# dog-qiuqiu/Yolo-FastestV2

Hardware: AMD Instinct MI355X
Metric: images/sec at 352x352 bs=256 per GPU (forward+decode+NMS) (higher is better)
Workload: dtype f32 tensors; contractions fp16x3 (two-term fp16 split operands on v_mfma_f32_16x16x32_f16, fp32 accumulate); depthwise/BN/ReLU/decode/NMS fp32 VALU; 1 GPU

## Files before the change

yolo_fastestv2_amd/csrc/yfv2_stage2h.hip:

```cpp
#include "yfv2_internal.h"
#include <atomic>
#include <utility>

typedef _Float16 yfv2_h8 __attribute__((ext_vector_type(8)));
typedef _Float16 yfv2_h2 __attribute__((ext_vector_type(2)));

namespace {

__device__ __forceinline__ float row_shr1(float v) {
  return __builtin_bit_cast(float, __builtin_amdgcn_update_dpp(0, __builtin_bit_cast(int, v), 0x111, 0xf, 0xf, true));
}
__device__ __forceinline__ float row_shl1(float v) {
  return __builtin_bit_cast(float, __builtin_amdgcn_update_dpp(0, __builtin_bit_cast(int, v), 0x101, 0xf, 0xf, true));
}
template <int K>
__device__ __forceinline__ float quad_mul(float tap4, float v) {
  return __builtin_bit_cast(float, __builtin_amdgcn_update_dpp(0, __builtin_bit_cast(int, tap4), K * 0x55, 0xf, 0xf, false)) * v;
}
#define YFV2_QP(n) "quad_perm:[%" #n ",%" #n ",%" #n ",%" #n "] row_mask:0xf bank_mask:0xf\n\t"
template <int K3, int K4, int K5, int K6, int K7, int K8>
__device__ __forceinline__ void quad_fmac6(float& a0, float& a1, float& a2, float t3, float t4, float t5, float t6, float t7, float t8,
                                           float u, float w) {
  asm("s_nop 1\n\tv_fmac_f32_dpp %0, %3, %9 " YFV2_QP(11) "v_fmac_f32_dpp %1, %4, %9 " YFV2_QP(12) "v_fmac_f32_dpp %2, %5, %9 " YFV2_QP(13)
      "v_fmac_f32_dpp %0, %6, %10 " YFV2_QP(14) "v_fmac_f32_dpp %1, %7, %10 " YFV2_QP(15) "v_fmac_f32_dpp %2, %8, %10 " YFV2_QP(16)
      : "+v"(a0), "+v"(a1), "+v"(a2)
      : "v"(t3), "v"(t4), "v"(t5), "v"(t6), "v"(t7), "v"(t8), "v"(u), "v"(w), "n"(K3), "n"(K4), "n"(K5), "n"(K6), "n"(K7), "n"(K8));
}
template <int KA, int KB, int KC>
__device__ __forceinline__ void quad_fmac3(float& s, float& q, float ta, float tb, float tc, float v0, float v1) {
  asm("s_nop 1\n\tv_fmac_f32_dpp %0, %2, %5 " YFV2_QP(7) "v_fmac_f32_dpp %1, %3, %6 " YFV2_QP(8) "v_fmac_f32_dpp %0, %4, %6 " YFV2_QP(9)
      : "+v"(s), "+v"(q) : "v"(ta), "v"(tb), "v"(tc), "v"(v0), "v"(v1), "n"(KA), "n"(KB), "n"(KC));
}
template <int KA>
__device__ __forceinline__ void quad_fmac1(float& s, float ta, float v) {
  asm("s_nop 1\n\tv_fmac_f32_dpp %0, %1, %2 " YFV2_QP(3) : "+v"(s) : "v"(ta), "v"(v), "n"(KA));
}
#undef YFV2_QP
__device__ __forceinline__ void dpp_src_ready(float& v) { asm volatile("s_nop 1" : "+v"(v)); }

__device__ __forceinline__ void split2(f32x2 v, unsigned& h1, unsigned& h2) {
  const yfv2_h2 t1 = __builtin_convertvector(v, yfv2_h2);
  const f32x2 r = v - __builtin_convertvector(t1, f32x2);
  const yfv2_h2 t2 = __builtin_convertvector(r, yfv2_h2);
  h1 = __builtin_bit_cast(unsigned, t1);
  h2 = __builtin_bit_cast(unsigned, t2);
}
__device__ __forceinline__ void pw_h3(const yfv2_h8 (&w)[2][2], const f32x2 (&in)[4], const f32x4 (&init)[2], f32x4 (&acc)[2], Yfv2Watch& watch) {
  u32x4 b1, b2;
#pragma unroll
  for (int k = 0; k < 4; ++k) { unsigned h1, h2; split2(in[k], h1, h2); b1[k] = h1; b2[k] = h2; }
  const yfv2_h8 x1 = __builtin_bit_cast(yfv2_h8, b1), x2 = __builtin_bit_cast(yfv2_h8, b2);
#pragma unroll
  for (int t = 0; t < 2; ++t) acc[t] = __builtin_amdgcn_mfma_f32_16x16x32_f16(w[t][0], x2, init[t], 0, 0, 0);
#pragma unroll
  for (int t = 0; t < 2; ++t) acc[t] = __builtin_amdgcn_mfma_f32_16x16x32_f16(w[t][1], x1, acc[t], 0, 0, 0);
#pragma unroll
  for (int t = 0; t < 2; ++t) acc[t] = __builtin_amdgcn_mfma_f32_16x16x32_f16(w[t][0], x1, acc[t], 0, 0, 0);
  watch.see(acc[0][0]);
}

}

constexpr int S1H_W1 = 0, S1H_W2 = 1024, S1H_TAPS = 2048, S1H_CST = 3200, S1H_OFFS = 3272;

__global__ __launch_bounds__(64, 3) void s1h_kernel(S1PxArgs a) {
  const int H = a.H, W = a.W;
  const int nstrips = a.nstrips, nb = a.nb, R = a.R;
  const int wpi = nstrips * nb;
  const int nwg = gridDim.x;
  const int wid = (nwg & 7) ? (int)blockIdx.x : (int)(blockIdx.x & 7) * (nwg >> 3) + (int)(blockIdx.x >> 3);
  const int b = __builtin_amdgcn_readfirstlane(wid / wpi), wi = __builtin_amdgcn_readfirstlane(wid - b * wpi);
  const int strip = wi % nstrips, band = wi / nstrips;
  const int lane = threadIdx.x, l = lane & 15, g = lane >> 4;
  const int x = 14 * strip + l;
  const bool xok = x < W;
  const bool st_lane = xok && (l > 0 || strip == 0) && (l < 15 || strip == nstrips - 1);
  const int y0 = band * R, y1 = min(H, y0 + R);
  constexpr int OOB = (int)0x80000000;

  __amdgpu_buffer_rsrc_t rsrc = __builtin_amdgcn_make_buffer_rsrc((void*)(a.act + (size_t)b * a.img_stride), 0, a.num_records, 0x00020000);
  const float* img = a.img16;
  yfv2_h8 w1[2][2], w2[2][2];
  {
    const u32x4* q = reinterpret_cast<const u32x4*>(img);
#pragma unroll
    for (int t = 0; t < 2; ++t)
#pragma unroll
      for (int k = 0; k < 2; ++k) {
        w1[t][k] = __builtin_bit_cast(yfv2_h8, q[(S1H_W1 / 4) + (t * 2 + k) * 64 + lane]);
        w2[t][k] = __builtin_bit_cast(yfv2_h8, q[(S1H_W2 / 4) + (t * 2 + k) * 64 + lane]);
      }
  }
  Yfv2Watch watch;
  float tq[18];
#pragma unroll
  for (int q = 0; q < 18; ++q) tq[q] = img[S1H_TAPS + q * 64 + lane];
  const f32x4 sh1[2] = {*reinterpret_cast<const f32x4*>(img + S1H_CST + 4 * g), *reinterpret_cast<const f32x4*>(img + S1H_CST + 16 + 4 * g)};
  const f32x4 bi2[2] = {*reinterpret_cast<const f32x4*>(img + S1H_CST + 32 + 4 * g), *reinterpret_cast<const f32x4*>(img + S1H_CST + 48 + 4 * g)};
  const float unscale2 = img[S1H_CST + 64];
  int soff[4], doff[4];
  {
    const int* po = reinterpret_cast<const int*>(img + S1H_OFFS);
#pragma unroll
    for (int k = 0; k < 4; ++k) {
      const int so = po[k * 64 + lane], dd = po[(4 + k) * 64 + lane];
      soff[k] = (xok && so != OOB) ? so + x * 8 : OOB;
      doff[k] = (st_lane && dd != OOB) ? dd + x * 8 : OOB;
    }
  }
  const int rowb = W * 8;

  auto load_row = [&](int r, f32x2 (&v)[4]) {
    const bool rok = r >= 0 && r < H;
#pragma unroll
// ... 795 lines not shown
    }(std::make_integer_sequence<int, 12>{});
  };

  f32x4 X[6], Y[6];
  float cxe[12], cxo[12], cte[12], cto[12];
  {
    const int iy = 2 * y0 - 1;
    load_row(iy, X);
    load_row(iy + 1, Y);
    columns(X, (xok && iy >= 0) ? __builtin_inff() : 0.f, cxe, cxo, cte, cto);
    load_row(iy + 2, X);
  }
  const float limx = xok ? __builtin_inff() : 0.f;
  for (int j = 0; j < R; ++j) {
    const int oy = y0 + j;
    float Sm[12], Qm[12], Sp[12], Qp[12], xe[12], xo[12], te[12], to[12];
    {
      float tm[27], tp[27]; ld_taps(tm, tp);
      acc_row(std::integral_constant<int, 0>{}, tm, cte, cto, Sm, Qm);
      acc_row(std::integral_constant<int, 0>{}, tp, cxe, cxo, Sp, Qp);
    }
    columns(Y, limx, xe, xo, te, to);
    {
      float tm[27], tp[27]; ld_taps(tm, tp);
      acc_row(std::integral_constant<int, 1>{}, tm, te, to, Sm, Qm);
      acc_row(std::integral_constant<int, 1>{}, tp, xe, xo, Sp, Qp);
    }
    __builtin_amdgcn_sched_barrier(0);
    load_row(2 * oy + 2, Y);
    __builtin_amdgcn_sched_barrier(0);
    columns(X, limx, cxe, cxo, cte, cto);
    {
      float tm[27], tp[27]; ld_taps(tm, tp);
      acc_row(std::integral_constant<int, 2>{}, tm, cte, cto, Sm, Qm);
      acc_row(std::integral_constant<int, 2>{}, tp, cxe, cxo, Sp, Qp);
    }
    __builtin_amdgcn_sched_barrier(0);
    load_row(2 * oy + 3, X);
    __builtin_amdgcn_sched_barrier(0);
    f32x2 dm[6], dp[6];
#pragma unroll
    for (int c = 0; c < 12; ++c) {
      dpp_src_ready(Qm[c]); dpp_src_ready(Qp[c]);
      dm[c >> 1][c & 1] = Sm[c] + row_shr1(Qm[c]);
      dp[c >> 1][c & 1] = Sp[c] + row_shr1(Qp[c]);
    }
    f32x4 am[3], ap[3];
    { f32x4 bip[3]; ld_c3(48, bip); pw_h3_48(WP, lane, dp, bip, ap, watch); }
    { f32x4 bi2[3]; ld_c3(96, bi2); pw_h3_48(W2, lane, dm, bi2, am, watch); }
    if (st_lane && oy < y1) {
      float* o = outp + (size_t)oy * OW * 96;
#pragma unroll
      for (int t = 0; t < 3; ++t) {
        f32x4 vp, vm;
#pragma unroll
        for (int e = 0; e < 4; ++e) { vp[e] = __builtin_fmaxf(ap[t][e], 0.f) * unscale_p; vm[e] = __builtin_fmaxf(am[t][e], 0.f) * unscale_2; }
        *reinterpret_cast<f32x4*>(o + 16 * t) = vp;
        *reinterpret_cast<f32x4*>(o + 48 + 16 * t) = vm;
      }
    }
  }
  watch.report(a.nonfinite);
#undef YFV2_TQ
#undef YFV2_TK
}

bool yfv2_s3h_supported(int H, int W) { return H >= 4 && W >= 4 && !(H & 1) && !(W & 1) && W / 2 <= 16 * 15; }

void yfv2_launch_s3h(const BlockS2Args& a0, hipStream_t s) {
  BlockS2Args a = a0;
  const int OH = a.H / 2, OW = a.W / 2;
  const int nstrips = OW <= 16 ? 1 : (OW - 1 + 14) / 15;
  int nb = (8 + nstrips - 1) / nstrips;
  if (nb > OH) nb = OH;
  a.R = (OH + nb - 1) / nb;
  nb = (OH + a.R - 1) / a.R;
  const int units = nstrips * nb;
  static std::atomic<unsigned long long> lds_ok{0};
  yfv2_allow_full_lds(reinterpret_cast<const void*>(&s3h2_kernel), lds_ok);
  YFV2_LAUNCH(s3h2_kernel, dim3(a.B * ((units + 3) / 4)), dim3(256), S3H2_FLOATS * sizeof(float), s, a);
}

constexpr int S4H_WFL = 9216, S4H_TM = 27648, S4H_TP = 27648 + 3456, S4H_CST = 27648 + 6912;

namespace {
__device__ __forceinline__ void pw_h3_96(const float* W, int lane, const f32x2 (&in)[12], const f32x4 (&init)[6], f32x4 (&acc)[6], Yfv2Watch& watch) {
  const u32x4* Wq = reinterpret_cast<const u32x4*>(W) + lane;
#pragma unroll
  for (int t = 0; t < 6; ++t) acc[t] = init[t];
#pragma unroll
  for (int c = 0; c < 3; ++c) {
    u32x4 b1, b2;
#pragma unroll
    for (int k = 0; k < 4; ++k) { unsigned h1, h2; split2(in[4 * c + k], h1, h2); b1[k] = h1; b2[k] = h2; }
    const yfv2_h8 x1 = __builtin_bit_cast(yfv2_h8, b1), x2 = __builtin_bit_cast(yfv2_h8, b2);
    yfv2_h8 wa[6][2];
#pragma unroll
    for (int t = 0; t < 6; ++t)
#pragma unroll
      for (int k = 0; k < 2; ++k) wa[t][k] = __builtin_bit_cast(yfv2_h8, Wq[((t * 3 + c) * 2 + k) * 64]);
#pragma unroll
    for (int t = 0; t < 6; ++t) acc[t] = __builtin_amdgcn_mfma_f32_16x16x32_f16(wa[t][0], x2, acc[t], 0, 0, 0);
#pragma unroll
    for (int t = 0; t < 6; ++t) acc[t] = __builtin_amdgcn_mfma_f32_16x16x32_f16(wa[t][1], x1, acc[t], 0, 0, 0);
#pragma unroll
    for (int t = 0; t < 6; ++t) acc[t] = __builtin_amdgcn_mfma_f32_16x16x32_f16(wa[t][0], x1, acc[t], 0, 0, 0);
  }
  watch.see(acc[0][0]);
}

template <bool MAIN>
__device__ __forceinline__ void s4h_body(const BlockS2Args& a, const float* lds, int b, int strip, int band, int R, int lane) {
  const int IH = a.H, IW = a.W, OH = IH >> 1, OW = IW >> 1;
  const int l = lane & 15, g = lane >> 4;
  const int ox = 15 * strip + l;
  const bool xok = ox < OW;
  const bool st_lane = xok && (l > 0 || strip == 0);
  const int y0 = band * R, y1 = min(OH, y0 + R);
  constexpr int OOB = (int)0x80000000;
  const float* img = a.img16;
  const float* W1 = lds; const float* WB = lds + (MAIN ? 2 : 1) * S4H_WFL;

  __amdgpu_buffer_rsrc_t rin = __builtin_amdgcn_make_buffer_rsrc((void*)(a.in + (size_t)b * 96 * IH * IW), 0, 96 * IH * IW * 4, 0x00020000);
  Yfv2Watch watch;
  float tq[54];
#pragma unroll
  for (int q = 0; q < 54; ++q) tq[q] = img[(MAIN ? S4H_TM : S4H_TP) + q * 64 + lane];
  f32x4 sh1[6], bib[6];
#pragma unroll
  for (int t = 0; t < 6; ++t) {
    sh1[t] = *reinterpret_cast<const f32x4*>(img + S4H_CST + 16 * t + 4 * g);
    bib[t] = *reinterpret_cast<const f32x4*>(img + S4H_CST + (MAIN ? 192 : 96) + 16 * t + 4 * g);
  }
  const float unscale = img[S4H_CST + 288 + (MAIN ? 1 : 0)];
  const int lbase = xok ? (2 * ox * 96 + 4 * g) * 4 : OOB;
  const int irowb = IW * 96 * 4;
  float* __restrict__ outp = a.out + ((size_t)b * OH * OW + (st_lane ? ox : 0)) * 192 + (MAIN ? 96 : 0) + 4 * g;

  auto load_row = [&](int iy, f32x4 (&X)[12]) {
    const bool rok = iy >= 0 && iy < IH;
    const int base = (rok && lbase != OOB) ? lbase + iy * irowb : OOB;
#pragma unroll
    for (int t = 0; t < 6; ++t) {
      X[t] = __builtin_bit_cast(f32x4, __builtin_amdgcn_raw_buffer_load_b128(rin, base, t * 64, 0));
      X[6 + t] = __builtin_bit_cast(f32x4, __builtin_amdgcn_raw_buffer_load_b128(rin, base, 384 + t * 64, 0));
    }
  };
  auto columns = [&](const f32x4 (&X)[12], float lim, float (&ve)[24], float (&vo)[24]) {
    if constexpr (MAIN) {
      f32x2 in[12];
      f32x4 acc[6];
#pragma unroll
      for (int t = 0; t < 6; ++t) { const f32x4 v = X[t] * 16.0f; in[2 * t] = (f32x2){v[0], v[1]}; in[2 * t + 1] = (f32x2){v[2], v[3]}; }
      pw_h3_96(W1, lane, in, sh1, acc, watch);
#pragma unroll
      for (int c = 0; c < 24; ++c) ve[c] = __builtin_amdgcn_fmed3f(acc[c >> 2][c & 3], 0.f, lim);
#pragma unroll
      for (int t = 0; t < 6; ++t) { const f32x4 v = X[6 + t] * 16.0f; in[2 * t] = (f32x2){v[0], v[1]}; in[2 * t + 1] = (f32x2){v[2], v[3]}; }
      pw_h3_96(W1, lane, in, sh1, acc, watch);
#pragma unroll
      for (int c = 0; c < 24; ++c) vo[c] = __builtin_amdgcn_fmed3f(acc[c >> 2][c & 3], 0.f, lim);
    } else {
#pragma unroll
      for (int t = 0; t < 6; ++t) {
        const f32x4 e = X[t] * 16.0f, o = X[6 + t] * 16.0f;
#pragma unroll
        for (int k = 0; k < 4; ++k) { ve[4 * t + k] = e[k]; vo[4 * t + k] = o[k]; }
      }
    }
  };
#define YFV2_TQ(c, t) tq[((c) * 9 + (t)) >> 2]
#define YFV2_TK(c, t) (((c) * 9 + (t)) & 3)
  auto acc_row = [&](auto dyc, const float (&v0)[24], const float (&v1)[24], float (&S)[24], float (&Q)[24]) {
    constexpr int DY = decltype(dyc)::value;
    [&]<int... Cs>(std::integer_sequence<int, Cs...>) {
      ((DY == 0 ? (void)(S[Cs] = quad_mul<YFV2_TK(Cs, 1)>(YFV2_TQ(Cs, 1), v0[Cs]), Q[Cs] = quad_mul<YFV2_TK(Cs, 0)>(YFV2_TQ(Cs, 0), v1[Cs]),
                         quad_fmac1<YFV2_TK(Cs, 2)>(S[Cs], YFV2_TQ(Cs, 2), v1[Cs]))
                : (void)quad_fmac3<YFV2_TK(Cs, DY * 3 + 1), YFV2_TK(Cs, DY * 3), YFV2_TK(Cs, DY * 3 + 2)>(
                      S[Cs], Q[Cs], YFV2_TQ(Cs, DY * 3 + 1), YFV2_TQ(Cs, DY * 3), YFV2_TQ(Cs, DY * 3 + 2), v0[Cs], v1[Cs])), ...);
    }(std::make_integer_sequence<int, 24>{});
  };

  f32x4 X[12];
  float ce[24], co[24];
  {
    const int iy = 2 * y0 - 1;
    load_row(iy, X);
    columns(X, (xok && iy >= 0) ? __builtin_inff() : 0.f, ce, co);
    load_row(iy + 1, X);
  }
  const float limx = xok ? __builtin_inff() : 0.f;
  for (int j = 0; j < R; ++j) {
    const int oy = y0 + j;
    float S[24], Q[24], ve[24], vo[24];
    acc_row(std::integral_constant<int, 0>{}, ce, co, S, Q);
    columns(X, limx, ve, vo);
    __builtin_amdgcn_sched_barrier(0);
    load_row(2 * oy + 1, X);
    __builtin_amdgcn_sched_barrier(0);
    acc_row(std::integral_constant<int, 1>{}, ve, vo, S, Q);
    columns(X, limx, ce, co);
    __builtin_amdgcn_sched_barrier(0);
    load_row(2 * oy + 2, X);
    __builtin_amdgcn_sched_barrier(0);
    acc_row(std::integral_constant<int, 2>{}, ce, co, S, Q);
    f32x2 d[12];
#pragma unroll
    for (int c = 0; c < 24; ++c) { dpp_src_ready(Q[c]); d[c >> 1][c & 1] = S[c] + row_shr1(Q[c]); }
    f32x4 acc[6];
    pw_h3_96(WB, lane, d, bib, acc, watch);
    if (st_lane && oy < y1) {
      float* o = outp + (size_t)oy * OW * 192;
#pragma unroll
      for (int t = 0; t < 6; ++t) {
        f32x4 v;
#pragma unroll
        for (int e = 0; e < 4; ++e) v[e] = __builtin_fmaxf(acc[t][e], 0.f) * unscale;
        *reinterpret_cast<f32x4*>(o + 16 * t) = v;
      }
    }
  }
  watch.report(a.nonfinite);
#undef YFV2_TQ
#undef YFV2_TK
}
}

__global__ __launch_bounds__(256, 1) void s4h_kernel(BlockS2Args a) {
  extern __shared__ __attribute__((aligned(16))) float lds[];
  const int OH = a.H >> 1, OW = a.W >> 1;
  const int nstrips = OW <= 16 ? 1 : (OW - 1 + 14) / 15;
  const int R = a.R, nb = (OH + R - 1) / R;
  const int units = nstrips * nb, wpi = (units + 1) >> 1;
  const int b = blockIdx.x / wpi, wi = blockIdx.x - b * wpi;
  const int tid = threadIdx.x, wave = tid >> 6;
  {
    const f32x4* src = reinterpret_cast<const f32x4*>(a.img16);
    f32x4* dst = reinterpret_cast<f32x4*>(lds);
#pragma unroll 1
    for (int r = 0; r < 3; ++r) {
      f32x4 tmp[9];
#pragma unroll
      for (int k = 0; k < 9; ++k) tmp[k] = src[(r * 9 + k) * 256 + tid];
#pragma unroll
      for (int k = 0; k < 9; ++k) dst[(r * 9 + k) * 256 + tid] = tmp[k];
    }
  }
  __syncthreads();
  if (a.s4_main_bands > 0) {
    const int mb = a.s4_main_bands;
    if (wave < mb) s4h_body<true>(a, lds, (int)blockIdx.x, 0, wave, (OH + mb - 1) / mb, tid & 63);
    else if (wave == 3) s4h_body<false>(a, lds, (int)blockIdx.x, 0, 0, OH, tid & 63);
    return;
  }
  const int uid = wi * 2 + (wave >> 1);
  if (uid >= units) return;
  const int strip = uid % nstrips, band = uid / nstrips;
  if (wave & 1) s4h_body<true>(a, lds, b, strip, band, R, tid & 63);
  else s4h_body<false>(a, lds, b, strip, band, R, tid & 63);
}

bool yfv2_s4h_supported(int H, int W) { return H >= 4 && W >= 4 && !(H & 1) && !(W & 1); }

void yfv2_launch_s4h(const BlockS2Args& a0, hipStream_t s) {
  BlockS2Args a = a0;
  const int OH = a.H / 2, OW = a.W / 2;
  const int nstrips = OW <= 16 ? 1 : (OW - 1 + 14) / 15;
  int nb = (2 + nstrips - 1) / nstrips;
  if (nb > OH) nb = OH;
  a.R = (OH + nb - 1) / nb;
  nb = (OH + a.R - 1) / a.R;
  const int units = nstrips * nb;
  static std::atomic<unsigned long long> lds_ok{0};
  yfv2_allow_full_lds(reinterpret_cast<const void*>(&s4h_kernel), lds_ok);
  a.s4_main_bands = (nstrips == 1 && OH >= 6) ? 3 : 0;
  if (a.s4_main_bands) { YFV2_LAUNCH(s4h_kernel, dim3(a.B), dim3(256), 3 * S4H_WFL * sizeof(float), s, a); return; }
  YFV2_LAUNCH(s4h_kernel, dim3(a.B * ((units + 1) / 2)), dim3(256), 3 * S4H_WFL * sizeof(float), s, a);
}
```

Measured before the change: 464,300 images/s.

## Restructure s4h kernel to 512 threads with LDS-resident taps and grouped pointwise

```diff
diff --git a/yolo_fastestv2_amd/csrc/yfv2_stage2h.hip b/yolo_fastestv2_amd/csrc/yfv2_stage2h.hip
--- a/yolo_fastestv2_amd/csrc/yfv2_stage2h.hip
+++ b/yolo_fastestv2_amd/csrc/yfv2_stage2h.hip
@@ -30,6 +30,11 @@
 __device__ __forceinline__ void quad_fmac3(float& s, float& q, float ta, float tb, float tc, float v0, float v1) {
   asm("s_nop 1\n\tv_fmac_f32_dpp %0, %2, %5 " YFV2_QP(7) "v_fmac_f32_dpp %1, %3, %6 " YFV2_QP(8) "v_fmac_f32_dpp %0, %4, %6 " YFV2_QP(9)
       : "+v"(s), "+v"(q) : "v"(ta), "v"(tb), "v"(tc), "v"(v0), "v"(v1), "n"(KA), "n"(KB), "n"(KC));
+}
+template <int KB, int KC>
+__device__ __forceinline__ void quad_fmac2(float& q, float& s, float tb, float tc, float v) {
+  asm("s_nop 1\n\tv_fmac_f32_dpp %0, %2, %4 " YFV2_QP(5) "v_fmac_f32_dpp %1, %3, %4 " YFV2_QP(6)
+      : "+v"(q), "+v"(s) : "v"(tb), "v"(tc), "v"(v), "n"(KB), "n"(KC));
 }
 template <int KA>
 __device__ __forceinline__ void quad_fmac1(float& s, float ta, float v) {
@@ -991,6 +996,7 @@
 }
 
 constexpr int S4H_WFL = 9216, S4H_TM = 27648, S4H_TP = 27648 + 3456, S4H_CST = 27648 + 6912;
+constexpr int S4H_TPITCH = 60, S4H_LT = 3 * S4H_WFL, S4H_LC = S4H_LT + 2 * 64 * S4H_TPITCH, S4H_LDS_FLOATS = S4H_LC + 292;
 
 namespace {
 __device__ __forceinline__ void pw_h3_96(const float* W, int lane, const f32x2 (&in)[12], const f32x4 (&init)[6], f32x4 (&acc)[6], Yfv2Watch& watch) {
@@ -1016,6 +1022,29 @@
     for (int t = 0; t < 6; ++t) acc[t] = __builtin_amdgcn_mfma_f32_16x16x32_f16(wa[t][0], x1, acc[t], 0, 0, 0);
   }
   watch.see(acc[0][0]);
+}
+template <int G>
+__device__ __forceinline__ void pw1_grp(const float* lds, int lane, const u32x4 (&b1)[3], const u32x4 (&b2)[3], f32x4 (&acc)[3], Yfv2Watch& watch) {
+  asm volatile("" ::: "memory");
+  const u32x4* Wq = reinterpret_cast<const u32x4*>(lds) + lane;
+#pragma unroll
+  for (int t = 0; t < 3; ++t) acc[t] = *reinterpret_cast<const f32x4*>(lds + S4H_LC + 16 * (3 * G + t) + 4 * (lane >> 4));
+#pragma unroll
+  for (int c = 0; c < 3; ++c) {
+    const yfv2_h8 x1 = __builtin_bit_cast(yfv2_h8, b1[c]), x2 = __builtin_bit_cast(yfv2_h8, b2[c]);
+    yfv2_h8 wa[3][2];
+#pragma unroll
+    for (int t = 0; t < 3; ++t)
+#pragma unroll
+      for (int k = 0; k < 2; ++k) wa[t][k] = __builtin_bit_cast(yfv2_h8, Wq[(((3 * G + t) * 3 + c) * 2 + k) * 64]);
+#pragma unroll
+    for (int t = 0; t < 3; ++t) acc[t] = __builtin_amdgcn_mfma_f32_16x16x32_f16(wa[t][0], x2, acc[t], 0, 0, 0);
+#pragma unroll
+    for (int t = 0; t < 3; ++t) acc[t] = __builtin_amdgcn_mfma_f32_16x16x32_f16(wa[t][1], x1, acc[t], 0, 0, 0);
+#pragma unroll
+    for (int t = 0; t < 3; ++t) acc[t] = __builtin_amdgcn_mfma_f32_16x16x32_f16(wa[t][0], x1, acc[t], 0, 0, 0);
+  }
+  if constexpr (G == 0) watch.see(acc[0][0]);
 }
 
 template <bool MAIN>
@@ -1026,99 +1055,131 @@
   const bool xok = ox < OW;
   const bool st_lane = xok && (l > 0 || strip == 0);
   const int y0 = band * R, y1 = min(OH, y0 + R);
+  if (y0 >= y1) return;
   constexpr int OOB = (int)0x80000000;
-  const float* img = a.img16;
-  const float* W1 = lds; const float* WB = lds + (MAIN ? 2 : 1) * S4H_WFL;
+  const float* WB = lds + (MAIN ? 2 : 1) * S4H_WFL;
+  const float* tapl = lds + S4H_LT + (MAIN ? 0 : 64 * S4H_TPITCH) + lane * S4H_TPITCH;
 
   __amdgpu_buffer_rsrc_t rin = __builtin_amdgcn_make_buffer_rsrc((void*)(a.in + (size_t)b * 96 * IH * IW), 0, 96 * IH * IW * 4, 0x00020000);
   Yfv2Watch watch;
-  float tq[54];
-#pragma unroll
-  for (int q = 0; q < 54; ++q) tq[q] = img[(MAIN ? S4H_TM : S4H_TP) + q * 64 + lane];
-  f32x4 sh1[6], bib[6];
-#pragma unroll
-  for (int t = 0; t < 6; ++t) {
-    sh1[t] = *reinterpret_cast<const f32x4*>(img + S4H_CST + 16 * t + 4 * g);
-    bib[t] = *reinterpret_cast<const f32x4*>(img + S4H_CST + (MAIN ? 192 : 96) + 16 * t + 4 * g);
-  }
-  const float unscale = img[S4H_CST + 288 + (MAIN ? 1 : 0)];
   const int lbase = xok ? (2 * ox * 96 + 4 * g) * 4 : OOB;
   const int irowb = IW * 96 * 4;
   float* __restrict__ outp = a.out + ((size_t)b * OH * OW + (st_lane ? ox : 0)) * 192 + (MAIN ? 96 : 0) + 4 * g;
 
-  auto load_row = [&](int iy, f32x4 (&X)[12]) {
+  auto load_col = [&](int iy, auto colc, f32x4 (&X)[6]) {
+    constexpr int COL = decltype(colc)::value;
     const bool rok = iy >= 0 && iy < IH;
     const int base = (rok && lbase != OOB) ? lbase + iy * irowb : OOB;
+    __builtin_amdgcn_sched_barrier(0);
+#pragma unroll
+    for (int t = 0; t < 6; ++t) X[t] = __builtin_bit_cast(f32x4, __builtin_amdgcn_raw_buffer_load_b128(rin, base, COL * 384 + t * 64, 0));
+    __builtin_amdgcn_sched_barrier(0);
+  };
+  u32x4 b1[3], b2[3];
+  float pv[24];
+  auto prep = [&](const f32x4 (&X)[6]) {
 #pragma unroll
     for (int t = 0; t < 6; ++t) {
-      X[t] = __builtin_bit_cast(f32x4, __builtin_amdgcn_raw_buffer_load_b128(rin, base, t * 64, 0));
-      X[6 + t] = __builtin_bit_cast(f32x4, __builtin_amdgcn_raw_buffer_load_b128(rin, base, 384 + t * 64, 0));
-    }
-  };
-  auto columns = [&](const f32x4 (&X)[12], float lim, float (&ve)[24], float (&vo)[24]) {
-    if constexpr (MAIN) {
-      f32x2 in[12];
-      f32x4 acc[6];
-#pragma unroll
-      for (int t = 0; t < 6; ++t) { const f32x4 v = X[t] * 16.0f; in[2 * t] = (f32x2){v[0], v[1]}; in[2 * t + 1] = (f32x2){v[2], v[3]}; }
-      pw_h3_96(W1, lane, in, sh1, acc, watch);
-#pragma unroll
-      for (int c = 0; c < 24; ++c) ve[c] = __builtin_amdgcn_fmed3f(acc[c >> 2][c & 3], 0.f, lim);
-#pragma unroll
-      for (int t = 0; t < 6; ++t) { const f32x4 v = X[6 + t] * 16.0f; in[2 * t] = (f32x2){v[0], v[1]}; in[2 * t + 1] = (f32x2){v[2], v[3]}; }
-      pw_h3_96(W1, lane, in, sh1, acc, watch);
-#pragma unroll
-      for (int c = 0; c < 24; ++c) vo[c] = __builtin_amdgcn_fmed3f(acc[c >> 2][c & 3], 0.f, lim);
-    } else {
-#pragma unroll
-      for (int t = 0; t < 6; ++t) {
-        const f32x4 e = X[t] * 16.0f, o = X[6 + t] * 16.0f;
-#pragma unroll
-        for (int k = 0; k < 4; ++k) { ve[4 * t + k] = e[k]; vo[4 * t + k] = o[k]; }
+      const f32x4 v = X[t] * 16.0f;
+      if constexpr (MAIN) {
+        unsigned h1, h2;
+        split2((f32x2){v[0], v[1]}, h1, h2); b1[t >> 1][2 * (t & 1)] = h1; b2[t >> 1][2 * (t & 1)] = h2;
+        split2((f32x2){v[2], v[3]}, h1, h2); b1[t >> 1][2 * (t & 1) + 1] = h1; b2[t >> 1][2 * (t & 1) + 1] = h2;
+      } else {
+#pragma unroll
+        for (int k = 0; k < 4; ++k) pv[4 * t + k] = v[k];
       }
     }
   };
-#define YFV2_TQ(c, t) tq[((c) * 9 + (t)) >> 2]
+  auto ld_taps = [&](auto gc, float (&T)[28]) {
+    constexpr int G = decltype(gc)::value;
+    asm volatile("" ::: "memory");
+    const f32x4* q = reinterpret_cast<const f32x4*>(tapl + 28 * G);
+#pragma unroll
+    for (int j = 0; j < 7; ++j) {
+      const f32x4 v = q[j];
+#pragma unroll
+      for (int e = 0; e < 4; ++e) T[4 * j + e] = v[e];
+    }
+  };
+#define YFV2_TQ(c, t) T[(((c) * 9 + (t)) >> 2) - 27 * G]
 #define YFV2_TK(c, t) (((c) * 9 + (t)) & 3)
-  auto acc_row = [&](auto dyc, const float (&v0)[24], const float (&v1)[24], float (&S)[24], float (&Q)[24]) {
-    constexpr int DY = decltype(dyc)::value;
-    [&]<int... Cs>(std::integer_sequence<int, Cs...>) {
-      ((DY == 0 ? (void)(S[Cs] = quad_mul<YFV2_TK(Cs, 1)>(YFV2_TQ(Cs, 1), v0[Cs]), Q[Cs] = quad_mul<YFV2_TK(Cs, 0)>(YFV2_TQ(Cs, 0), v1[Cs]),
-                         quad_fmac1<YFV2_TK(Cs, 2)>(S[Cs], YFV2_TQ(Cs, 2), v1[Cs]))
-                : (void)quad_fmac3<YFV2_TK(Cs, DY * 3 + 1), YFV2_TK(Cs, DY * 3), YFV2_TK(Cs, DY * 3 + 2)>(
-                      S[Cs], Q[Cs], YFV2_TQ(Cs, DY * 3 + 1), YFV2_TQ(Cs, DY * 3), YFV2_TQ(Cs, DY * 3 + 2), v0[Cs], v1[Cs])), ...);
-    }(std::make_integer_sequence<int, 24>{});
-  };
-
-  f32x4 X[12];
+  auto dy0 = [&](auto gc, const float (&ce)[24], const float (&co)[24], float (&S)[24], float (&Q)[24]) {
+    constexpr int G = decltype(gc)::value;
+    float T[28]; ld_taps(gc, T);
+    [&]<int... Is>(std::integer_sequence<int, Is...>) {
+      ((S[12 * G + Is] = quad_mul<YFV2_TK(12 * G + Is, 1)>(YFV2_TQ(12 * G + Is, 1), ce[12 * G + Is]),
+        Q[12 * G + Is] = quad_mul<YFV2_TK(12 * G + Is, 0)>(YFV2_TQ(12 * G + Is, 0), co[12 * G + Is]),
+        quad_fmac1<YFV2_TK(12 * G + Is, 2)>(S[12 * G + Is], YFV2_TQ(12 * G + Is, 2), co[12 * G + Is])), ...);
+    }(std::make_integer_sequence<int, 12>{});
+  };
+  auto work = [&](auto dyc, auto colc, float lim, float (&S)[24], float (&Q)[24], float (&keep)[24]) {
+    constexpr int DY = decltype(dyc)::value, COL = decltype(colc)::value;
+    [&]<int... Gs>(std::integer_sequence<int, Gs...>) {
+      ([&] {
+        constexpr int G = Gs;
+        float v[12];
+        if constexpr (MAIN) {
+          f32x4 acc[3];
+          pw1_grp<G>(lds, lane, b1, b2, acc, watch);
+#pragma unroll
+          for (int i = 0; i < 12; ++i) v[i] = __builtin_amdgcn_fmed3f(acc[i >> 2][i & 3], 0.f, lim);
+        } else {
+#pragma unroll
+          for (int i = 0; i < 12; ++i) v[i] = pv[12 * G + i];
+        }
+        if constexpr (DY == 2 || DY < 0) {
+#pragma unroll
+          for (int i = 0; i < 12; ++i) keep[12 * G + i] = v[i];
+        }
+        if constexpr (DY > 0) {
+          float T[28]; ld_taps(std::integral_constant<int, G>{}, T);
+          [&]<int... Is>(std::integer_sequence<int, Is...>) {
+            ((COL == 0 ? (void)quad_fmac1<YFV2_TK(12 * G + Is, DY * 3 + 1)>(S[12 * G + Is], YFV2_TQ(12 * G + Is, DY * 3 + 1), v[Is])
+                       : (void)quad_fmac2<YFV2_TK(12 * G + Is, DY * 3), YFV2_TK(12 * G + Is, DY * 3 + 2)>(
+                             Q[12 * G + Is], S[12 * G + Is], YFV2_TQ(12 * G + Is, DY * 3), YFV2_TQ(12 * G + Is, DY * 3 + 2), v[Is])), ...);
+          }(std::make_integer_sequence<int, 12>{});
+        }
+      }(), ...);
+    }(std::integer_sequence<int, 0, 1>{});
+  };
+  using I0 = std::integral_constant<int, 0>; using I1 = std::integral_constant<int, 1>; using I2 = std::integral_constant<int, 2>;
+  using IM = std::integral_constant<int, -1>;
+
+  f32x4 X[6];
   float ce[24], co[24];
+  const float limx = xok ? __builtin_inff() : 0.f;
   {
     const int iy = 2 * y0 - 1;
-    load_row(iy, X);
-    columns(X, (xok && iy >= 0) ? __builtin_inff() : 0.f, ce, co);
-    load_row(iy + 1, X);
-  }
-  const float limx = xok ? __builtin_inff() : 0.f;
-  for (int j = 0; j < R; ++j) {
-    const int oy = y0 + j;
-    float S[24], Q[24], ve[24], vo[24];
-    acc_row(std::integral_constant<int, 0>{}, ce, co, S, Q);
-    columns(X, limx, ve, vo);
-    __builtin_amdgcn_sched_barrier(0);
-    load_row(2 * oy + 1, X);
-    __builtin_amdgcn_sched_barrier(0);
-    acc_row(std::integral_constant<int, 1>{}, ve, vo, S, Q);
-    columns(X, limx, ce, co);
-    __builtin_amdgcn_sched_barrier(0);
-    load_row(2 * oy + 2, X);
-    __builtin_amdgcn_sched_barrier(0);
-    acc_row(std::integral_constant<int, 2>{}, ce, co, S, Q);
+    const float lim0 = (xok && iy >= 0) ? __builtin_inff() : 0.f;
+    load_col(iy, I0{}, X);
+    prep(X); load_col(iy, I1{}, X);
+    work(IM{}, I0{}, lim0, ce, co, ce);
+    prep(X); load_col(iy + 1, I0{}, X);
+    work(IM{}, I1{}, lim0, ce, co, co);
+  }
+  for (int oy = y0; oy < y1; ++oy) {
+    float S[24], Q[24];
+    dy0(I0{}, ce, co, S, Q);
+    dy0(I1{}, ce, co, S, Q);
+    prep(X); load_col(2 * oy, I1{}, X);
+    work(I1{}, I0{}, limx, S, Q, ce);
+    prep(X); load_col(2 * oy + 1, I0{}, X);
+    work(I1{}, I1{}, limx, S, Q, co);
+    prep(X); load_col(2 * oy + 1, I1{}, X);
+    work(I2{}, I0{}, limx, S, Q, ce);
+    prep(X); load_col(2 * oy + 2, I0{}, X);
+    work(I2{}, I1{}, limx, S, Q, co);
     f32x2 d[12];
 #pragma unroll
     for (int c = 0; c < 24; ++c) { dpp_src_ready(Q[c]); d[c >> 1][c & 1] = S[c] + row_shr1(Q[c]); }
-    f32x4 acc[6];
+    f32x4 acc[6], bib[6];
+    asm volatile("" ::: "memory");
+#pragma unroll
+    for (int t = 0; t < 6; ++t) bib[t] = *reinterpret_cast<const f32x4*>(lds + S4H_LC + (MAIN ? 192 : 96) + 16 * t + 4 * g);
+    const float unscale = lds[S4H_LC + 288 + (MAIN ? 1 : 0)];
     pw_h3_96(WB, lane, d, bib, acc, watch);
-    if (st_lane && oy < y1) {
+    if (st_lane) {
       float* o = outp + (size_t)oy * OW * 192;
 #pragma unroll
       for (int t = 0; t < 6; ++t) {
@@ -1135,34 +1196,43 @@
 }
 }
 
-__global__ __launch_bounds__(256, 1) void s4h_kernel(BlockS2Args a) {
+__global__ __launch_bounds__(512) void s4h_kernel(BlockS2Args a) {
   extern __shared__ __attribute__((aligned(16))) float lds[];
   const int OH = a.H >> 1, OW = a.W >> 1;
   const int nstrips = OW <= 16 ? 1 : (OW - 1 + 14) / 15;
   const int R = a.R, nb = (OH + R - 1) / R;
-  const int units = nstrips * nb, wpi = (units + 1) >> 1;
+  const int units = nstrips * nb, wpi = (units + 3) >> 2;
   const int b = blockIdx.x / wpi, wi = blockIdx.x - b * wpi;
   const int tid = threadIdx.x, wave = tid >> 6;
   {
     const f32x4* src = reinterpret_cast<const f32x4*>(a.img16);
     f32x4* dst = reinterpret_cast<f32x4*>(lds);
 #pragma unroll 1
-    for (int r = 0; r < 3; ++r) {
-      f32x4 tmp[9];
-#pragma unroll
-      for (int k = 0; k < 9; ++k) tmp[k] = src[(r * 9 + k) * 256 + tid];
-#pragma unroll
-      for (int k = 0; k < 9; ++k) dst[(r * 9 + k) * 256 + tid] = tmp[k];
-    }
+    for (int r = 0; r < 2; ++r) {
+      f32x4 tmp[7];
+#pragma unroll
+      for (int k = 0; k < 7; ++k) { const int i = (r * 7 + k) * 512 + tid; tmp[k] = i < 3 * S4H_WFL / 4 ? src[i] : (f32x4){0.f, 0.f, 0.f, 0.f}; }
+#pragma unroll
+      for (int k = 0; k < 7; ++k) { const int i = (r * 7 + k) * 512 + tid; if (i < 3 * S4H_WFL / 4) dst[i] = tmp[k]; }
+    }
+    float tv[14];
+#pragma unroll
+    for (int j = 0; j < 14; ++j) { const int e = tid + 512 * j; tv[j] = e < 2 * 54 * 64 ? a.img16[S4H_TM + e] : 0.f; }
+    const float cv = tid < 292 ? a.img16[S4H_CST + tid] : 0.f;
+#pragma unroll
+    for (int j = 0; j < 14; ++j) {
+      const int e = tid + 512 * j, role = e / (54 * 64), q = (e >> 6) - 54 * role;
+      if (e < 2 * 54 * 64) lds[S4H_LT + (role * 64 + (e & 63)) * S4H_TPITCH + q + (q >= 27 ? 1 : 0)] = tv[j];
+    }
+    if (tid < 292) lds[S4H_LC + tid] = cv;
   }
   __syncthreads();
   if (a.s4_main_bands > 0) {
-    const int mb = a.s4_main_bands;
-    if (wave < mb) s4h_body<true>(a, lds, (int)blockIdx.x, 0, wave, (OH + mb - 1) / mb, tid & 63);
-    else if (wave == 3) s4h_body<false>(a, lds, (int)blockIdx.x, 0, 0, OH, tid & 63);
+    if (wave < 6) s4h_body<true>(a, lds, (int)blockIdx.x, 0, wave < 3 ? wave : wave == 3 ? 5 : wave - 1, (OH + 5) / 6, tid & 63);
+    else s4h_body<false>(a, lds, (int)blockIdx.x, 0, 7 - wave, (OH + 1) / 2, tid & 63);
     return;
   }
-  const int uid = wi * 2 + (wave >> 1);
+  const int uid = wi * 4 + (wave >> 1);
   if (uid >= units) return;
   const int strip = uid % nstrips, band = uid / nstrips;
   if (wave & 1) s4h_body<true>(a, lds, b, strip, band, R, tid & 63);
@@ -1175,14 +1245,14 @@
   BlockS2Args a = a0;
   const int OH = a.H / 2, OW = a.W / 2;
   const int nstrips = OW <= 16 ? 1 : (OW - 1 + 14) / 15;
-  int nb = (2 + nstrips - 1) / nstrips;
+  int nb = (4 + nstrips - 1) / nstrips;
   if (nb > OH) nb = OH;
   a.R = (OH + nb - 1) / nb;
   nb = (OH + a.R - 1) / a.R;
   const int units = nstrips * nb;
   static std::atomic<unsigned long long> lds_ok{0};
   yfv2_allow_full_lds(reinterpret_cast<const void*>(&s4h_kernel), lds_ok);
-  a.s4_main_bands = (nstrips == 1 && OH >= 6) ? 3 : 0;
-  if (a.s4_main_bands) { YFV2_LAUNCH(s4h_kernel, dim3(a.B), dim3(256), 3 * S4H_WFL * sizeof(float), s, a); return; }
-  YFV2_LAUNCH(s4h_kernel, dim3(a.B * ((units + 1) / 2)), dim3(256), 3 * S4H_WFL * sizeof(float), s, a);
-}
+  a.s4_main_bands = (nstrips == 1 && OH >= 6) ? 6 : 0;
+  if (a.s4_main_bands) { YFV2_LAUNCH(s4h_kernel, dim3(a.B), dim3(512), S4H_LDS_FLOATS * sizeof(float), s, a); return; }
+  YFV2_LAUNCH(s4h_kernel, dim3(a.B * ((units + 3) / 4)), dim3(512), S4H_LDS_FLOATS * sizeof(float), s, a);
+}
```

Result: no change. 468,400 images/s, median of 6 (+0.9%).

## Add 8-wave s4h kernel splitting main branch across bands and channel halves

Applied to the files above, without the earlier changes.

```diff
diff --git a/yolo_fastestv2_amd/csrc/yfv2_stage2h.hip b/yolo_fastestv2_amd/csrc/yfv2_stage2h.hip
--- a/yolo_fastestv2_amd/csrc/yfv2_stage2h.hip
+++ b/yolo_fastestv2_amd/csrc/yfv2_stage2h.hip
@@ -1169,12 +1169,295 @@
   else s4h_body<false>(a, lds, b, strip, band, R, tid & 63);
 }
 
+constexpr int S4W_XCH = 3 * S4H_WFL, S4W_XHALF = 768;
+constexpr int S4W_BIAS = S4W_XCH + 3 * 2 * 2 * S4W_XHALF;
+constexpr int S4W_LDS_FLOATS = S4W_BIAS + 96;
+
+namespace {
+__device__ __forceinline__ void pw_h3_96x3(const u32x4* Wq, const u32x4 (&b1)[3], const u32x4 (&b2)[3], const f32x4 (&init)[3], f32x4 (&acc)[3],
+                                           Yfv2Watch& watch) {
+#pragma unroll
+  for (int t = 0; t < 3; ++t) acc[t] = init[t];
+#pragma unroll
+  for (int c = 0; c < 3; ++c) {
+    const yfv2_h8 x1 = __builtin_bit_cast(yfv2_h8, b1[c]), x2 = __builtin_bit_cast(yfv2_h8, b2[c]);
+    yfv2_h8 wa[3][2];
+#pragma unroll
+    for (int t = 0; t < 3; ++t)
+#pragma unroll
+      for (int k = 0; k < 2; ++k) wa[t][k] = __builtin_bit_cast(yfv2_h8, Wq[((t * 3 + c) * 2 + k) * 64]);
+#pragma unroll
+    for (int t = 0; t < 3; ++t) acc[t] = __builtin_amdgcn_mfma_f32_16x16x32_f16(wa[t][0], x2, acc[t], 0, 0, 0);
+#pragma unroll
+    for (int t = 0; t < 3; ++t) acc[t] = __builtin_amdgcn_mfma_f32_16x16x32_f16(wa[t][1], x1, acc[t], 0, 0, 0);
+#pragma unroll
+    for (int t = 0; t < 3; ++t) acc[t] = __builtin_amdgcn_mfma_f32_16x16x32_f16(wa[t][0], x1, acc[t], 0, 0, 0);
+  }
+  watch.see(acc[0][0]);
+}
+
+__device__ __forceinline__ void s4w_main(const BlockS2Args& a, float* lds, int b, int band, int half, int NB, int lane) {
+  const int IH = a.H, IW = a.W, OH = IH >> 1, OW = IW >> 1;
+  const int l = lane & 15, g = lane >> 4;
+  const bool xok = l < OW;
+  const int y0 = band * NB, y1 = min(OH, y0 + NB);
+  constexpr int OOB = (int)0x80000000;
+  const float* img = a.img16;
+  const u32x4* W1q = reinterpret_cast<const u32x4*>(lds) + half * 1152 + lane;
+  const u32x4* W2q = reinterpret_cast<const u32x4*>(lds + 2 * S4H_WFL) + half * 1152 + lane;
+  u32x4* xq = reinterpret_cast<u32x4*>(lds + S4W_XCH + band * 4 * S4W_XHALF) + lane;
+
+  __amdgpu_buffer_rsrc_t rin = __builtin_amdgcn_make_buffer_rsrc((void*)(a.in + (size_t)b * 96 * IH * IW), 0, 96 * IH * IW * 4, 0x00020000);
+  Yfv2Watch watch;
+  float tq[27];
+#pragma unroll
+  for (int q = 0; q < 27; ++q) tq[q] = img[S4H_TM + (27 * half + q) * 64 + lane];
+  f32x4 sh1[3], bib[3];
+#pragma unroll
+  for (int t = 0; t < 3; ++t) {
+    sh1[t] = *reinterpret_cast<const f32x4*>(img + S4H_CST + 16 * (3 * half + t) + 4 * g);
+    bib[t] = *reinterpret_cast<const f32x4*>(img + S4H_CST + 192 + 16 * (3 * half + t) + 4 * g);
+  }
+  const float unscale = img[S4H_CST + 289];
+  const int lbase = xok ? (2 * l * 96 + 4 * g) * 4 : OOB;
+  const int irowb = IW * 96 * 4;
+  float* __restrict__ outp = a.out + ((size_t)b * OH * OW + (xok ? l : 0)) * 192 + 96 + 16 * 3 * half + 4 * g;
+
+  auto load_row = [&](int iy, f32x4 (&X)[12]) {
+    const bool rok = iy >= 0 && iy < IH;
+    const int base = (rok && lbase != OOB) ? lbase + iy * irowb : OOB;
+#pragma unroll
+    for (int t = 0; t < 6; ++t) {
+      X[t] = __builtin_bit_cast(f32x4, __builtin_amdgcn_raw_buffer_load_b128(rin, base, t * 64, 0));
+      X[6 + t] = __builtin_bit_cast(f32x4, __builtin_amdgcn_raw_buffer_load_b128(rin, base, 384 + t * 64, 0));
+    }
+  };
+  auto column = [&](const f32x4* X6, float lim, float (&v)[12]) {
+    u32x4 b1[3], b2[3];
+#pragma unroll
+    for (int t = 0; t < 6; ++t) {
+      const f32x4 x = X6[t] * 16.0f;
+      unsigned h1, h2;
+      split2((f32x2){x[0], x[1]}, h1, h2); b1[t >> 1][2 * (t & 1)] = h1; b2[t >> 1][2 * (t & 1)] = h2;
+      split2((f32x2){x[2], x[3]}, h1, h2); b1[t >> 1][2 * (t & 1) + 1] = h1; b2[t >> 1][2 * (t & 1) + 1] = h2;
+    }
+    f32x4 acc[3];
+    pw_h3_96x3(W1q, b1, b2, sh1, acc, watch);
+#pragma unroll
+    for (int c = 0; c < 12; ++c) v[c] = __builtin_amdgcn_fmed3f(acc[c >> 2][c & 3], 0.f, lim);
+  };
+#define YFV2_TQ(c, t) tq[((c) * 9 + (t)) >> 2]
+#define YFV2_TK(c, t) (((c) * 9 + (t)) & 3)
+  auto acc_row = [&](auto dyc, const float (&v0)[12], const float (&v1)[12], float (&S)[12], float (&Q)[12]) {
+    constexpr int DY = decltype(dyc)::value;
+    [&]<int... Cs>(std::integer_sequence<int, Cs...>) {
+      ((DY == 0 ? (void)(S[Cs] = quad_mul<YFV2_TK(Cs, 1)>(YFV2_TQ(Cs, 1), v0[Cs]), Q[Cs] = quad_mul<YFV2_TK(Cs, 0)>(YFV2_TQ(Cs, 0), v1[Cs]),
+                         quad_fmac1<YFV2_TK(Cs, 2)>(S[Cs], YFV2_TQ(Cs, 2), v1[Cs]))
+                : (void)quad_fmac3<YFV2_TK(Cs, DY * 3 + 1), YFV2_TK(Cs, DY * 3), YFV2_TK(Cs, DY * 3 + 2)>(
+                      S[Cs], Q[Cs], YFV2_TQ(Cs, DY * 3 + 1), YFV2_TQ(Cs, DY * 3), YFV2_TQ(Cs, DY * 3 + 2), v0[Cs], v1[Cs])), ...);
+    }(std::make_integer_sequence<int, 12>{});
+  };
+
+  const float limx = xok ? __builtin_inff() : 0.f;
+  f32x4 X[12];
+  float ce[12], co[12];
+  if (y0 > 0) {
+    load_row(2 * y0 - 1, X);
+    column(X, limx, ce);
+    column(X + 6, limx, co);
+  } else {
+#pragma unroll
+    for (int c = 0; c < 12; ++c) ce[c] = co[c] = 0.f;
+  }
+  load_row(2 * y0, X);
+  for (int j = 0; j < NB; ++j) {
+    const int oy = y0 + j;
+    const bool live = oy < y1;
+    u32x4* xw = xq + ((j & 1) * 2 + half) * 192;
+    if (live) {
+      float S[12], Q[12], ve[12], vo[12];
+      acc_row(std::integral_constant<int, 0>{}, ce, co, S, Q);
+      column(X, limx, ve);
+      column(X + 6, limx, vo);
+      __builtin_amdgcn_sched_barrier(0);
+      load_row(2 * oy + 1, X);
+      __builtin_amdgcn_sched_barrier(0);
+      acc_row(std::integral_constant<int, 1>{}, ve, vo, S, Q);
+      column(X, limx, ce);
+      column(X + 6, limx, co);
+      __builtin_amdgcn_sched_barrier(0);
+      load_row(2 * oy + 2, X);
+      __builtin_amdgcn_sched_barrier(0);
+      acc_row(std::integral_constant<int, 2>{}, ce, co, S, Q);
+      unsigned h1[6], h2[6];
+#pragma unroll
+      for (int p = 0; p < 6; ++p) {
+        dpp_src_ready(Q[2 * p]); dpp_src_ready(Q[2 * p + 1]);
+        split2((f32x2){S[2 * p] + row_shr1(Q[2 * p]), S[2 * p + 1] + row_shr1(Q[2 * p + 1])}, h1[p], h2[p]);
+      }
+      u32x4 o0, o1, o2;
+#pragma unroll
+      for (int k = 0; k < 4; ++k) { o0[k] = half ? h1[2 + k] : h1[k]; o1[k] = half ? h2[2 + k] : h2[k]; }
+      o2[0] = half ? h1[0] : h1[4]; o2[1] = half ? h1[1] : h1[5]; o2[2] = half ? h2[0] : h2[4]; o2[3] = half ? h2[1] : h2[5];
+      xw[0] = o0; xw[64] = o1; xw[128] = o2;
+    }
+    __syncthreads();
+    if (live) {
+      const u32x4* x0 = xq + (j & 1) * 2 * 192;
+      u32x4 b1[3], b2[3];
+      b1[0] = x0[0]; b2[0] = x0[64];
+      const u32x4 p0 = x0[128], p1 = x0[192 + 128];
+      b1[1] = (u32x4){p0[0], p0[1], p1[0], p1[1]}; b2[1] = (u32x4){p0[2], p0[3], p1[2], p1[3]};
+      b1[2] = x0[192]; b2[2] = x0[192 + 64];
+      f32x4 acc[3];
+      pw_h3_96x3(W2q, b1, b2, bib, acc, watch);
+      if (xok) {
+        float* o = outp + (size_t)oy * OW * 192;
+#pragma unroll
+        for (int t = 0; t < 3; ++t) {
+          f32x4 v;
+#pragma unroll
+          for (int e = 0; e < 4; ++e) v[e] = __builtin_fmaxf(acc[t][e], 0.f) * unscale;
+          *reinterpret_cast<f32x4*>(o + 16 * t) = v;
+        }
+      }
+    }
+  }
+  watch.report(a.nonfinite);
+#undef YFV2_TQ
+#undef YFV2_TK
+}
+
+__device__ __forceinline__ void s4w_proj(const BlockS2Args& a, const float* lds, int b, int band, int RP, int NB, int lane) {
+  const int IH = a.H, IW = a.W, OH = IH >> 1, OW = IW >> 1;
+  const int l = lane & 15, g = lane >> 4;
+  const bool xok = l < OW;
+  const int y0 = band * RP, y1 = min(OH, y0 + RP);
+  constexpr int OOB = (int)0x80000000;
+  const float* img = a.img16;
+  const float* WP = lds + S4H_WFL;
+  __amdgpu_buffer_rsrc_t rin = __builtin_amdgcn_make_buffer_rsrc((void*)(a.in + (size_t)b * 96 * IH * IW), 0, 96 * IH * IW * 4, 0x00020000);
+  Yfv2Watch watch;
+  float tq[54];
+#pragma unroll
+  for (int q = 0; q < 54; ++q) tq[q] = img[S4H_TP + q * 64 + lane];
+  const float unscale = img[S4H_CST + 288];
+  const int lbase = xok ? (2 * l * 96 + 4 * g) * 4 : OOB;
+  const int irowb = IW * 96 * 4;
+  float* __restrict__ outp = a.out + ((size_t)b * OH * OW + (xok ? l : 0)) * 192 + 4 * g;
+
+  auto load_row = [&](int iy, f32x4 (&X)[12]) {
+    const bool rok = iy >= 0 && iy < IH;
+    const int base = (rok && lbase != OOB) ? lbase + iy * irowb : OOB;
+#pragma unroll
+    for (int t = 0; t < 6; ++t) {
+      X[t] = __builtin_bit_cast(f32x4, __builtin_amdgcn_raw_buffer_load_b128(rin, base, t * 64, 0));
+      X[6 + t] = __builtin_bit_cast(f32x4, __builtin_amdgcn_raw_buffer_load_b128(rin, base, 384 + t * 64, 0));
+    }
+  };
+#define YFV2_TQ(c, t) tq[((c) * 9 + (t)) >> 2]
+#define YFV2_TK(c, t) (((c) * 9 + (t)) & 3)
+  auto acc_row = [&](auto dyc, const f32x4 (&X)[12], float (&S)[24], float (&Q)[24]) {
+    constexpr int DY = decltype(dyc)::value;
+    [&]<int... Cs>(std::integer_sequence<int, Cs...>) {
+      ((DY == 0 ? (void)(S[Cs] = quad_mul<YFV2_TK(Cs, 1)>(YFV2_TQ(Cs, 1), X[Cs >> 2][Cs & 3] * 16.0f), Q[Cs] = quad_mul<YFV2_TK(Cs, 0)>(YFV2_TQ(Cs, 0), X[6 + (Cs >> 2)][Cs & 3] * 16.0f),
+                         quad_fmac1<YFV2_TK(Cs, 2)>(S[Cs], YFV2_TQ(Cs, 2), X[6 + (Cs >> 2)][Cs & 3] * 16.0f))
+                : (void)quad_fmac3<YFV2_TK(Cs, DY * 3 + 1), YFV2_TK(Cs, DY * 3), YFV2_TK(Cs, DY * 3 + 2)>(
+                      S[Cs], Q[Cs], YFV2_TQ(Cs, DY * 3 + 1), YFV2_TQ(Cs, DY * 3), YFV2_TQ(Cs, DY * 3 + 2), X[Cs >> 2][Cs & 3] * 16.0f, X[6 + (Cs >> 2)][Cs & 3] * 16.0f)), ...);
+    }(std::make_integer_sequence<int, 24>{});
+  };
+
+  f32x4 XO[12], XE[12];
+  load_row(2 * y0 - 1, XO);
+  load_row(2 * y0, XE);
+  int done = 0;
+  for (int j = 0; j < RP; ++j) {
+    const int oy = y0 + j;
+    float S[24], Q[24];
+    acc_row(std::integral_constant<int, 0>{}, XO, S, Q);
+    __builtin_amdgcn_sched_barrier(0);
+    load_row(2 * oy + 1, XO);
+    __builtin_amdgcn_sched_barrier(0);
+    acc_row(std::integral_constant<int, 1>{}, XE, S, Q);
+    __builtin_amdgcn_sched_barrier(0);
+    load_row(2 * oy + 2, XE);
+    __builtin_amdgcn_sched_barrier(0);
+    acc_row(std::integral_constant<int, 2>{}, XO, S, Q);
+    f32x2 d[12];
+#pragma unroll
+    for (int c = 0; c < 24; ++c) { dpp_src_ready(Q[c]); d[c >> 1][c & 1] = S[c] + row_shr1(Q[c]); }
+    f32x4 bib[6], acc[6];
+#pragma unroll
+    for (int t = 0; t < 6; ++t) bib[t] = *reinterpret_cast<const f32x4*>(lds + S4W_BIAS + 16 * t + 4 * g);
+    pw_h3_96(WP, lane, d, bib, acc, watch);
+    if (xok && oy < y1) {
+      float* o = outp + (size_t)oy * OW * 192;
+#pragma unroll
+      for (int t = 0; t < 6; ++t) {
+        f32x4 v;
+#pragma unroll
+        for (int e = 0; e < 4; ++e) v[e] = __builtin_fmaxf(acc[t][e], 0.f) * unscale;
+        *reinterpret_cast<f32x4*>(o + 16 * t) = v;
+      }
+    }
+    while (done < NB && (j + 1) * NB >= (done + 1) * RP) { __syncthreads(); ++done; }
+  }
+  watch.report(a.nonfinite);
+#undef YFV2_TQ
+#undef YFV2_TK
+}
+}
+
+__global__ __launch_bounds__(512, 1) void s4h_kernel_w8(BlockS2Args a) {
+  extern __shared__ __attribute__((aligned(16))) float lds[];
+  const int OH = a.H >> 1;
+  const int tid = threadIdx.x, wave = tid >> 6;
+  {
+    const f32x4* src = reinterpret_cast<const f32x4*>(a.img16);
+    f32x4* dst = reinterpret_cast<f32x4*>(lds);
+#pragma unroll 1
+    for (int r = 0; r < 2; ++r) {
+      f32x4 tmp[7];
+#pragma unroll
+      for (int k = 0; k < 7; ++k) { const int i = (r * 7 + k) * 512 + tid; if (i < 3 * S4H_WFL / 4) tmp[k] = src[i]; }
+#pragma unroll
+      for (int k = 0; k < 7; ++k) { const int i = (r * 7 + k) * 512 + tid; if (i < 3 * S4H_WFL / 4) dst[i] = tmp[k]; }
+    }
+  }
+  if (tid < 96) lds[S4W_BIAS + tid] = a.img16[S4H_CST + 96 + tid];
+  __syncthreads();
+  const int NB = (OH + 2) / 3;
+  if (wave < 6) s4w_main(a, lds, (int)blockIdx.x, wave >> 1, wave & 1, NB, tid & 63);
+  else s4w_proj(a, lds, (int)blockIdx.x, 7 - wave, (OH + 1) >> 1, NB, tid & 63);
+}
+
 bool yfv2_s4h_supported(int H, int W) { return H >= 4 && W >= 4 && !(H & 1) && !(W & 1); }
+
+namespace {
+bool s4w_lds_granted() {
+  static std::atomic<unsigned long long> asked{0}, granted{0};
+  int dev = 0;
+  if (hipGetDevice(&dev) != hipSuccess || dev < 0 || dev > 63) dev = 0;
+  const unsigned long long bit = 1ull << dev;
+  if (!(asked.load(std::memory_order_acquire) & bit)) {
+    if (hipFuncSetAttribute(reinterpret_cast<const void*>(&s4h_kernel_w8), hipFuncAttributeMaxDynamicSharedMemorySize, S4W_LDS_FLOATS * (int)sizeof(float)) == hipSuccess)
+      granted.fetch_or(bit, std::memory_order_relaxed);
+    else
+      (void)hipGetLastError();
+    asked.fetch_or(bit, std::memory_order_release);
+  }
+  return (granted.load(std::memory_order_relaxed) & bit) != 0;
+}
+}
 
 void yfv2_launch_s4h(const BlockS2Args& a0, hipStream_t s) {
   BlockS2Args a = a0;
   const int OH = a.H / 2, OW = a.W / 2;
   const int nstrips = OW <= 16 ? 1 : (OW - 1 + 14) / 15;
+  if (nstrips == 1 && OH >= 6 && s4w_lds_granted()) {
+    YFV2_LAUNCH(s4h_kernel_w8, dim3(a.B), dim3(512), S4W_LDS_FLOATS * sizeof(float), s, a);
+    return;
+  }
   int nb = (2 + nstrips - 1) / nstrips;
   if (nb > OH) nb = OH;
   a.R = (OH + nb - 1) / nb;
```

Measured after the change: 463,700 images/s before, 465,600 images/s after, median of 4. About the same (+0.4%).
